# volcengine/veScale

Hardware: AMD Instinct MI355X
Metric: tokens/sec (whole node) Llama-3-8B veScale-FSDP (higher is better)
Workload: dtype bf16; 1 GPU; model=llama3_8b, global_batch=4, seq_len=8192, parallelism=fsdp1, activation_checkpointing=False, hipgraph=True

## Files before the change

### vescale_amd/ops/csrc/attention_bwd2.hip

```cpp
#include "fa32_common.h"

#define FB_D FF_D
#define FB_OWN 32
#define FB_WAVES 8
#define FB_TILE (FB_OWN * FB_WAVES)
#define FB_OTH 64
#define FB_THREADS (FB_WAVES * 64)

extern "C" __global__ void __launch_bounds__(256)
fa_bwd_preprocess(const unsigned short* __restrict__ dout,
                  const unsigned short* __restrict__ o,
                  float* __restrict__ delta, int64_t rows, int Hq, int S, int bshd) {
  const int sub = threadIdx.x & 15;
  int64_t row = (int64_t)blockIdx.x * 16 + (threadIdx.x >> 4);
  const int64_t stride = (int64_t)gridDim.x * 16;
  for (; row < rows; row += stride) {
    const unsigned short* pd = dout + row * FB_D + sub * 8;
    const unsigned short* po = o + row * FB_D + sub * 8;
    ff_shortx8 a = *reinterpret_cast<const ff_shortx8*>(pd);
    ff_shortx8 b = *reinterpret_cast<const ff_shortx8*>(po);
    float s = 0.f;
#pragma unroll
    for (int j = 0; j < 8; ++j)
      s += bf16_to_f32((unsigned short)a[j]) * bf16_to_f32((unsigned short)b[j]);
// ... 3 lines not shown
    int64_t drow = row;
    if (bshd) {
      const unsigned r = (unsigned)row, bs = r / (unsigned)Hq, h = r - bs * (unsigned)Hq;
      const unsigned bi = bs / (unsigned)S, sq = bs - bi * (unsigned)S;
      drow = ((int64_t)bi * Hq + h) * S + sq;
    }
    if (sub == 0) delta[drow] = s;
  }
}

extern "C" __global__ void __launch_bounds__(256)
fa_bwd_reduce_gqa(const unsigned short* __restrict__ part,
                  unsigned short* __restrict__ out,
                  int B, int Hq, int Hkv, int64_t SD) {
  int group = Hq / Hkv;
  int64_t total = (int64_t)B * Hkv * SD;
  int64_t i0 = (int64_t)(blockIdx.x * 256 + threadIdx.x) * 8;
  int64_t stride = (int64_t)gridDim.x * 256 * 8;
  for (int64_t i = i0; i < total; i += stride) {
    int64_t bh = i / SD;
    int64_t off = i % SD;
    int64_t b = bh / Hkv;
    int64_t hk = bh % Hkv;
    float acc[8] = {0, 0, 0, 0, 0, 0, 0, 0};
#pragma unroll 4
    for (int g = 0; g < group; ++g) {
      const unsigned short* p =
          part + ((b * Hq + hk * group + g) * SD) + off;
      ff_shortx8 v = *reinterpret_cast<const ff_shortx8*>(p);
#pragma unroll
      for (int j = 0; j < 8; ++j) acc[j] += bf16_to_f32((unsigned short)v[j]);
    }
    ff_shortx8 o;
#pragma unroll
    for (int j = 0; j < 8; ++j) o[j] = (short)f32_to_bf16(acc[j]);
    *reinterpret_cast<ff_shortx8*>(out + i) = o;
  }
}

extern "C" __global__ void __launch_bounds__(FB_THREADS, 2)
fa2_dq_bf16(const unsigned short* __restrict__ q,
            const unsigned short* __restrict__ k,
            const unsigned short* __restrict__ v,
            const unsigned short* __restrict__ dout,
            const float* __restrict__ lse,
            const float* __restrict__ delta,
            unsigned short* __restrict__ dq,
            int B, int Hq, int Hkv, int S, float scale, int bshd) {
  __shared__ unsigned short lk[FB_OTH * FB_D];
  __shared__ unsigned short lv[FB_OTH * FB_D];
  __shared__ unsigned short ldo[FB_TILE * FB_D];

  const ff_ctx c = ff_prologue(Hq, Hkv, S);
  const int tid = c.tid, wave = c.wave, l31 = c.l31, half = c.half;
  const int qt = (int)gridDim.x - 1 - c.tile;
  const int64_t qbase = c.qbase, kbase = c.kbase;
  const int q0 = qt * FB_TILE + wave * FB_OWN;
  const int my_q = q0 + l31;
  const float scale2 = scale * FF_LOG2E;

  const int64_t lrow = c.rbase + my_q;
  const float lse2 = lse[lrow] * FF_LOG2E;
  const float dlt = delta[lrow];

  ff_shortx8 qf[8];
  ff_row_frags(q + qbase + (int64_t)my_q * FB_D, qf, half);
  const ff_rows dorow = ff_o_rows(c, Hq, S, bshd);
  ff_stage_rows<FB_TILE, FB_THREADS>(
      dout + dorow.base + (int64_t)qt * FB_TILE * dorow.stride, dorow.stride, ldo, tid);

  ff_floatx16 dqacc[4];
#pragma unroll
  for (int i = 0; i < 4; ++i) dqacc[i] = (ff_floatx16)(0.f);

  const int last_kv = min((qt + 1) * (FB_TILE / FB_OTH), S / FB_OTH);
  const unsigned short* kg = k + kbase;
  const unsigned short* vg = v + kbase;

  for (int jkv = 0; jkv < last_kv; ++jkv) {
    const int kv0 = jkv * FB_OTH;
    const bool active = (kv0 <= q0 + FB_OWN - 1);
    const bool need_mask = (kv0 + FB_OTH - 1 > q0);
    __syncthreads();
    ff_stage<FB_OTH, FB_THREADS>(kg + (int64_t)kv0 * FB_D, lk, tid);
    ff_stage<FB_OTH, FB_THREADS>(vg + (int64_t)kv0 * FB_D, lv, tid);
    __syncthreads();

    if (active) {
      ff_floatx16 st[2], dp[2];
#pragma unroll
      for (int s2 = 0; s2 < 2; ++s2) {
        st[s2] = (ff_floatx16)(0.f);
        dp[s2] = (ff_floatx16)(0.f);
      }
#pragma unroll
      for (int s2 = 0; s2 < 2; ++s2)
#pragma unroll
        for (int ks = 0; ks < 8; ++ks) {
          ff_shortx8 kfr = ff_afrag(lk, s2, ks, l31, half);
          st[s2] = __builtin_amdgcn_mfma_f32_32x32x16_bf16(kfr, qf[ks], st[s2], 0, 0, 0);
          ff_shortx8 vfr = ff_afrag(lv, s2, ks, l31, half);
          ff_shortx8 dof = ff_bfrag(ldo, wave * FB_OWN + l31, ks, half);
          dp[s2] = __builtin_amdgcn_mfma_f32_32x32x16_bf16(vfr, dof, dp[s2], 0, 0, 0);
        }
#pragma unroll
      for (int s2 = 0; s2 < 2; ++s2)
#pragma unroll
        for (int r = 0; r < 16; ++r) {
          int kv = ff_drow(kv0 + s2 * 32, r, half);
          float x = st[s2][r] * scale2 - lse2;
          if (need_mask && kv > my_q) x = -INFINITY;
          float p = __builtin_amdgcn_exp2f(x);
          st[s2][r] = p * (dp[s2][r] - dlt);
        }
      ff_shortx8 pb[4];
      ff_relayout(st, pb, half);
#pragma unroll
      for (int ds = 0; ds < 4; ++ds) {
        ff_shortx4 t[4][2];
        ff_tr_read8(lk, ds, tid, l31, half, t);
#pragma unroll
        for (int ks = 0; ks < 4; ++ks)
          dqacc[ds] = __builtin_amdgcn_mfma_f32_32x32x16_bf16(
              ff_cat(t[ks][0], t[ks][1]), pb[ks], dqacc[ds], 0, 0, 0);
      }
    }
  }

  ff_store_row(dq + qbase + (int64_t)my_q * FB_D, dqacc, scale, half);
}

template <bool DK>
DEV void fa2_dv_dk_t(const unsigned short* __restrict__ q,
                     const unsigned short* __restrict__ k,
                     const unsigned short* __restrict__ v,
                     const unsigned short* __restrict__ dout,
                     const float* __restrict__ lse,
                     const float* __restrict__ delta,
                     unsigned short* __restrict__ out_part,
                     int Hq, int Hkv, int S, float scale, int bshd) {
  __shared__ unsigned short lq[FB_OTH * FB_D];
  __shared__ unsigned short ldo[FB_OTH * FB_D];
  __shared__ float llse[FB_OTH];
  __shared__ float ldelta[FB_OTH];

  const ff_ctx c = ff_prologue(Hq, Hkv, S);
  const int tid = c.tid, wave = c.wave, l31 = c.l31, half = c.half;
  const int64_t qbase = c.qbase, kbase = c.kbase;
  const int kvB = c.tile * FB_TILE;
  const int kv0w = kvB + wave * FB_OWN;
  const int my_kv = kv0w + l31;
  const float scale2 = scale * FF_LOG2E;

  ff_shortx8 kf[8], vf[DK ? 8 : 1];
  {
    const unsigned short* kg = k + kbase + (int64_t)my_kv * FB_D;
    const unsigned short* vg = DK ? v + kbase + (int64_t)my_kv * FB_D : nullptr;
#pragma unroll
    for (int ks = 0; ks < 8; ++ks) {
      kf[ks] = ff_row_frag(kg, ks, half);
      if constexpr (DK) vf[ks] = ff_row_frag(vg, ks, half);
    }
  }

  ff_floatx16 acc[4];
#pragma unroll
  for (int i = 0; i < 4; ++i) acc[i] = (ff_floatx16)(0.f);

  const int jq0 = kvB / FB_OTH;
  const int n_jq = S / FB_OTH;
  const float* lseg = lse + c.rbase;
  const float* dltg = DK ? delta + c.rbase : nullptr;
  const ff_rows dorow = ff_o_rows(c, Hq, S, bshd);

  for (int jq = jq0; jq < n_jq; ++jq) {
    const int qt0 = jq * FB_OTH;
    const bool active = (qt0 + FB_OTH - 1 >= kv0w);
    const bool need_mask = (qt0 < kv0w + FB_OWN - 1);
    __syncthreads();
    ff_stage<FB_OTH, FB_THREADS>(q + qbase + (int64_t)qt0 * FB_D, lq, tid);
    ff_stage_rows<FB_OTH, FB_THREADS>(dout + dorow.base + (int64_t)qt0 * dorow.stride,
                                      dorow.stride, ldo, tid);
    if (tid < FB_OTH) {
      llse[tid] = lseg[qt0 + tid] * FF_LOG2E;
      if constexpr (DK) ldelta[tid] = dltg[qt0 + tid];
    }
    __syncthreads();

    if (active) {
      ff_floatx16 st[2], dp[DK ? 2 : 1];
#pragma unroll
      for (int s2 = 0; s2 < 2; ++s2) {
        st[s2] = (ff_floatx16)(0.f);
        if constexpr (DK) dp[s2] = (ff_floatx16)(0.f);
      }
#pragma unroll
      for (int s2 = 0; s2 < 2; ++s2)
#pragma unroll
        for (int ks = 0; ks < 8; ++ks) {
          ff_shortx8 qfr = ff_afrag(lq, s2, ks, l31, half);
          st[s2] = __builtin_amdgcn_mfma_f32_32x32x16_bf16(qfr, kf[ks], st[s2], 0, 0, 0);
          if constexpr (DK) {
            ff_shortx8 dofr = ff_afrag(ldo, s2, ks, l31, half);
            dp[s2] = __builtin_amdgcn_mfma_f32_32x32x16_bf16(dofr, vf[ks], dp[s2], 0, 0, 0);
          }
        }
#pragma unroll
      for (int s2 = 0; s2 < 2; ++s2)
#pragma unroll
        for (int r = 0; r < 16; ++r) {
          int qrow = ff_drow(s2 * 32, r, half);
          float x = st[s2][r] * scale2 - llse[qrow];
          if (need_mask && qt0 + qrow < my_kv) x = -INFINITY;
          float p = __builtin_amdgcn_exp2f(x);
          if constexpr (DK) st[s2][r] = p * (dp[s2][r] - ldelta[qrow]);
          else st[s2][r] = p;
        }
      ff_shortx8 pb[4];
      ff_relayout(st, pb, half);
#pragma unroll
      for (int ds = 0; ds < 4; ++ds) {
        ff_shortx4 t[4][2];
        ff_tr_read8(DK ? lq : ldo, ds, tid, l31, half, t);
#pragma unroll
        for (int ks = 0; ks < 4; ++ks)
          acc[ds] = __builtin_amdgcn_mfma_f32_32x32x16_bf16(
              ff_cat(t[ks][0], t[ks][1]), pb[ks], acc[ds], 0, 0, 0);
      }
    }
  }

  unsigned short* og = out_part + qbase + (int64_t)my_kv * FB_D;
  ff_store_row<DK>(og, acc, scale, half);
}

extern "C" __global__ void __launch_bounds__(FB_THREADS, 2)
fa2_dv_bf16(const unsigned short* __restrict__ q,
            const unsigned short* __restrict__ k,
            const unsigned short* __restrict__ dout,
            const float* __restrict__ lse,
            unsigned short* __restrict__ dv_part,
            int B, int Hq, int Hkv, int S, float scale, int bshd) {
  fa2_dv_dk_t<false>(q, k, nullptr, dout, lse, nullptr, dv_part, Hq, Hkv, S, scale, bshd);
}

extern "C" __global__ void __launch_bounds__(FB_THREADS, 2)
fa2_dk_bf16(const unsigned short* __restrict__ q,
            const unsigned short* __restrict__ k,
            const unsigned short* __restrict__ v,
            const unsigned short* __restrict__ dout,
            const float* __restrict__ lse,
            const float* __restrict__ delta,
            unsigned short* __restrict__ dk_part,
            int B, int Hq, int Hkv, int S, float scale, int bshd) {
  fa2_dv_dk_t<true>(q, k, v, dout, lse, delta, dk_part, Hq, Hkv, S, scale, bshd);
}

#define FD_WAVES 4
#define FD_THREADS (FD_WAVES * 64)
#define FD_TILE (FD_WAVES * FB_OWN)

extern "C" __global__ void __launch_bounds__(FD_THREADS, 1)
fa2_dvdk_bf16(const unsigned short* __restrict__ q,
              const unsigned short* __restrict__ k,
              const unsigned short* __restrict__ v,
              const unsigned short* __restrict__ dout,
              const float* __restrict__ lse,
              const float* __restrict__ delta,
              unsigned short* __restrict__ dv_part,
              unsigned short* __restrict__ dk_part,
              int B, int Hq, int Hkv, int S, float scale) {
  __shared__ unsigned short lq[FB_OTH * FB_D];
// ... 23 lines not shown

  {
    const unsigned short* kg = k + kbase + (int64_t)kvB * FB_D;
    const unsigned short* vg = v + kbase + (int64_t)kvB * FB_D;
#pragma unroll
    for (int j = 0; j < FF_STAGE_CHUNKS(FD_TILE, FD_THREADS); ++j) {
      const int e = ff_chunk<FD_THREADS>(j, tid);
      ff_chunk_store(ff_chunk_load(kg, e), lk, e);
      ff_chunk_store(ff_chunk_load(vg, e), lv, e);
    }
  }

  ff_floatx16 dvacc[4], dkacc[4];
#pragma unroll
  for (int i = 0; i < 4; ++i) {
    dvacc[i] = (ff_floatx16)(0.f);
    dkacc[i] = (ff_floatx16)(0.f);
  }

  const int jq0 = kvB / FB_OTH;
  const int n_jq = S / FB_OTH;
  const float* lseg = lse + ((int64_t)b * Hq + h) * S;
  const float* dltg = delta + ((int64_t)b * Hq + h) * S;

  for (int jq = jq0; jq < n_jq; ++jq) {
    const int qt0 = jq * FB_OTH;
    const bool active = (qt0 + FB_OTH - 1 >= kv0w);
    const bool need_mask = (qt0 < kv0w + FB_OWN - 1);
    __syncthreads();
    ff_stage<FB_OTH, FD_THREADS>(q + qbase + (int64_t)qt0 * FB_D, lq, tid);
    ff_stage<FB_OTH, FD_THREADS>(dout + qbase + (int64_t)qt0 * FB_D, ldo, tid);
    const float lse_reg = lseg[qt0 + lane] * FF_LOG2E;
    const float dlt_reg = dltg[qt0 + lane];
    __syncthreads();

    if (active) {
      ff_floatx16 st[2], dp[2];
#pragma unroll
      for (int s2 = 0; s2 < 2; ++s2) {
        st[s2] = (ff_floatx16)(0.f);
        dp[s2] = (ff_floatx16)(0.f);
      }
#pragma unroll
      for (int s2 = 0; s2 < 2; ++s2)
#pragma unroll
        for (int ks = 0; ks < 8; ++ks) {
          ff_shortx8 kfr = ff_bfrag(lk, myrow, ks, half);
          ff_shortx8 qfr = ff_afrag(lq, s2, ks, l31, half);
          st[s2] = __builtin_amdgcn_mfma_f32_32x32x16_bf16(qfr, kfr, st[s2], 0, 0, 0);
          ff_shortx8 vfr = ff_bfrag(lv, myrow, ks, half);
          ff_shortx8 dofr = ff_afrag(ldo, s2, ks, l31, half);
          dp[s2] = __builtin_amdgcn_mfma_f32_32x32x16_bf16(dofr, vfr, dp[s2], 0, 0, 0);
        }
#pragma unroll
      for (int s2 = 0; s2 < 2; ++s2)
#pragma unroll
        for (int r = 0; r < 16; ++r) {
          int qrow = ff_drow(s2 * 32, r, half);
          float l2 = __int_as_float(
              __builtin_amdgcn_ds_bpermute(qrow * 4, __float_as_int(lse_reg)));
          float x = st[s2][r] * scale2 - l2;
          if (need_mask && qt0 + qrow < my_kv) x = -INFINITY;
          st[s2][r] = __builtin_amdgcn_exp2f(x);
        }
      {
        ff_shortx8 pb[4];
        ff_relayout(st, pb, half);
#pragma unroll
        for (int ds = 0; ds < 4; ++ds) {
          ff_shortx4 t[4][2];
          ff_tr_read8(ldo, ds, tid, l31, half, t);
#pragma unroll
          for (int ks = 0; ks < 4; ++ks)
            dvacc[ds] = __builtin_amdgcn_mfma_f32_32x32x16_bf16(
                ff_cat(t[ks][0], t[ks][1]), pb[ks], dvacc[ds], 0, 0, 0);
        }
      }
#pragma unroll
      for (int s2 = 0; s2 < 2; ++s2)
#pragma unroll
        for (int r = 0; r < 16; ++r) {
          int qrow = ff_drow(s2 * 32, r, half);
          float dl = __int_as_float(
              __builtin_amdgcn_ds_bpermute(qrow * 4, __float_as_int(dlt_reg)));
          st[s2][r] = st[s2][r] * (dp[s2][r] - dl);
        }
      {
        ff_shortx8 pb[4];
        ff_relayout(st, pb, half);
#pragma unroll
        for (int ds = 0; ds < 4; ++ds) {
          ff_shortx4 t[4][2];
          ff_tr_read8(lq, ds, tid, l31, half, t);
#pragma unroll
          for (int ks = 0; ks < 4; ++ks)
            dkacc[ds] = __builtin_amdgcn_mfma_f32_32x32x16_bf16(
                ff_cat(t[ks][0], t[ks][1]), pb[ks], dkacc[ds], 0, 0, 0);
        }
      }
    }
  }

  unsigned short* ogv = dv_part + qbase + (int64_t)my_kv * FB_D;
  unsigned short* ogk = dk_part + qbase + (int64_t)my_kv * FB_D;
#pragma unroll
  for (int ds = 0; ds < 4; ++ds)
#pragma unroll
    for (int r = 0; r < 16; ++r) {
      ff_store_elem(ogv, ds, r, half, dvacc[ds][r]);
      ff_store_elem(ogk, ds, r, half, dkacc[ds][r] * scale);
    }
}
```

### vescale_amd/ops/csrc/attention_fwd.hip

```cpp
#include "fa32_common.h"

#define FF_QBLK 32
#define FF_WAVES 4
#define FF_QTILE (FF_QBLK * FF_WAVES)
#define FF_KV 64
#define FF_THREADS (FF_WAVES * 64)
#define FF_CHUNKS FF_STAGE_CHUNKS(FF_KV, FF_THREADS)

template <int MODE>
DEV void fa_fwd_t(const unsigned short* __restrict__ q,
            const unsigned short* __restrict__ k,
            const unsigned short* __restrict__ v,
            unsigned short* __restrict__ out,
            float* __restrict__ lse,
            int B, int Hq, int Hkv, int S, float scale, int out_bshd) {
  __shared__ unsigned short lk[2][FF_KV * FF_D];
  __shared__ unsigned short lv[2][FF_KV * FF_D];

  const ff_ctx c = ff_prologue(Hq, Hkv, S);
  const int tid = c.tid, lane = c.lane, l31 = c.l31, half = c.half;
  const int qt = c.tile;
  const int q0 = qt * FF_QTILE + c.wave * FF_QBLK;
  const int my_q = q0 + l31;
  const float scale2 = (MODE == 5) ? scale : scale * FF_LOG2E;

  ff_shortx8 qf[8];
  ff_row_frags(q + c.qbase + (int64_t)my_q * FF_D, qf, half);

  float m_run = -INFINITY;
  float l_run = 0.f;
  ff_floatx16 oacc[4];
#pragma unroll
  for (int i = 0; i < 4; ++i) oacc[i] = (ff_floatx16)(0.f);

  const int n_kv = (qt + 1) * (FF_QTILE / FF_KV);
  const int last_kv = min(n_kv, S / FF_KV);

  const unsigned short* kg = k + c.kbase;
  const unsigned short* vg = v + c.kbase;
  ff_shortx8 kreg[FF_CHUNKS], vreg[FF_CHUNKS];
#pragma unroll
  for (int j = 0; j < FF_CHUNKS; ++j) {
    const int e = ff_chunk<FF_THREADS>(j, tid);
    kreg[j] = ff_chunk_load(kg, e);
    vreg[j] = ff_chunk_load(vg, e);
  }
#pragma unroll
  for (int j = 0; j < FF_CHUNKS; ++j) {
    const int e = ff_chunk<FF_THREADS>(j, tid);
    ff_chunk_store(kreg[j], lk[0], e);
    ff_chunk_store(vreg[j], lv[0], e);
  }
  __syncthreads();

  for (int jkv = 0; jkv < last_kv; ++jkv) {
    const int kv0 = jkv * FF_KV;
    const int buf = jkv & 1;
    const bool have_next = (jkv + 1 < last_kv);
    const bool active = (MODE == 4) || (kv0 <= q0 + FF_QBLK - 1);
    const bool need_mask = (MODE == 4) || (kv0 + FF_KV - 1 > q0);
    if (have_next) {
      const unsigned short* kn = kg + (int64_t)(kv0 + FF_KV) * FF_D;
      const unsigned short* vn = vg + (int64_t)(kv0 + FF_KV) * FF_D;
#pragma unroll
      for (int j = 0; j < FF_CHUNKS; ++j) {
        const int e = ff_chunk<FF_THREADS>(j, tid);
        kreg[j] = ff_chunk_load(kn, e);
        vreg[j] = ff_chunk_load(vn, e);
      }
    }

    if (active) {
    ff_floatx16 st[2];
#pragma unroll
    for (int s2 = 0; s2 < 2; ++s2) st[s2] = (ff_floatx16)(MODE == 3 ? 1e-3f : 0.f);
    if constexpr (MODE != 3)
#pragma unroll
    for (int s2 = 0; s2 < 2; ++s2) {
#pragma unroll
      for (int ks = 0; ks < 8; ++ks) {
        ff_shortx8 kf = ff_afrag(lk[buf], s2, ks, l31, half);
        st[s2] = __builtin_amdgcn_mfma_f32_32x32x16_bf16(kf, qf[ks], st[s2], 0, 0, 0);
      }
    }

    if constexpr (MODE == 1 || MODE == 3) {
      l_run += 1.f; m_run = 0.f;
    } else {
    float pmax = -INFINITY;
    if (need_mask) {
#pragma unroll
      for (int s2 = 0; s2 < 2; ++s2)
#pragma unroll
        for (int r = 0; r < 16; ++r) {
          int kv = ff_drow(kv0 + s2 * 32, r, half);
          float x = (kv <= my_q) ? st[s2][r] * scale2 : -INFINITY;
          st[s2][r] = x;
          pmax = fmaxf(pmax, x);
        }
    } else {
#pragma unroll
      for (int s2 = 0; s2 < 2; ++s2)
#pragma unroll
        for (int r = 0; r < 16; ++r) {
          float x = st[s2][r] * scale2;
          st[s2][r] = x;
          pmax = fmaxf(pmax, x);
        }
    }
    pmax = fmaxf(pmax, __int_as_float(ff_swap_other(__float_as_int(pmax), half)));
    float m_new = fmaxf(m_run, pmax);
    bool dead = false;
    if constexpr (MODE == 4) dead = (m_new == -INFINITY);
    float corr;
    if constexpr (MODE == 5) corr = __expf(m_run - m_new);
    else corr = __builtin_amdgcn_exp2f(m_run - m_new);
    if (dead) { corr = 1.f; m_new = m_run; }
    float psum = 0.f;
#pragma unroll
    for (int s2 = 0; s2 < 2; ++s2)
#pragma unroll
      for (int r = 0; r < 16; ++r) {
        float p;
        if (dead) p = 0.f;
        else if constexpr (MODE == 5) p = (st[s2][r] == -INFINITY) ? 0.f : __expf(st[s2][r] - m_new);
        else p = __builtin_amdgcn_exp2f(st[s2][r] - m_new);
        st[s2][r] = p;
        psum += p;
      }
    psum += __int_as_float(ff_swap_other(__float_as_int(psum), half));
    l_run = l_run * corr + psum;
    m_run = m_new;

#pragma unroll
    for (int ds = 0; ds < 4; ++ds)
#pragma unroll
      for (int r = 0; r < 16; ++r) oacc[ds][r] *= corr;
    }

    if constexpr (MODE == 2) {
#pragma unroll
      for (int r = 0; r < 16; ++r) oacc[0][r] += st[0][r] + st[1][r];
    } else {
    ff_shortx8 pb[4];
    ff_relayout(st, pb, half);
#pragma unroll
    for (int ds = 0; ds < 4; ++ds) {
      ff_shortx4 t[4][2];
      ff_tr_read8(lv[buf], ds, lane, l31, half, t);
#pragma unroll
      for (int ks = 0; ks < 4; ++ks)
        oacc[ds] = __builtin_amdgcn_mfma_f32_32x32x16_bf16(
            ff_cat(t[ks][0], t[ks][1]), pb[ks], oacc[ds], 0, 0, 0);
    }
    }
    }

    if (have_next) {
#pragma unroll
      for (int j = 0; j < FF_CHUNKS; ++j) {
        const int e = ff_chunk<FF_THREADS>(j, tid);
        ff_chunk_store(kreg[j], lk[buf ^ 1], e);
        ff_chunk_store(vreg[j], lv[buf ^ 1], e);
      }
    }
    __syncthreads();
  }

  float inv_l = (l_run > 0.f) ? 1.0f / l_run : 0.f;
  const ff_rows orow = ff_o_rows(c, Hq, S, out_bshd);
  ff_store_row(out + orow.base + (int64_t)my_q * orow.stride, oacc, inv_l, half);
  if (half == 0)
    lse[c.rbase + my_q] = m_run * (MODE == 5 ? 1.0f : FF_LN2) + __logf(l_run);
}

extern "C" __global__ void __launch_bounds__(FF_THREADS, 2)
fa_fwd_bf16(const unsigned short* q, const unsigned short* k,
            const unsigned short* v, unsigned short* out, float* lse,
            int B, int Hq, int Hkv, int S, float scale, int out_bshd) {
  fa_fwd_t<0>(q, k, v, out, lse, B, Hq, Hkv, S, scale, out_bshd);
}
extern "C" __global__ void __launch_bounds__(FF_THREADS, 2)
fa_fwd_bf16_ab1(const unsigned short* q, const unsigned short* k,
                const unsigned short* v, unsigned short* out, float* lse,
                int B, int Hq, int Hkv, int S, float scale, int out_bshd) {
  fa_fwd_t<1>(q, k, v, out, lse, B, Hq, Hkv, S, scale, out_bshd);
}
extern "C" __global__ void __launch_bounds__(FF_THREADS, 2)
fa_fwd_bf16_ab2(const unsigned short* q, const unsigned short* k,
                const unsigned short* v, unsigned short* out, float* lse,
                int B, int Hq, int Hkv, int S, float scale, int out_bshd) {
  fa_fwd_t<2>(q, k, v, out, lse, B, Hq, Hkv, S, scale, out_bshd);
}
extern "C" __global__ void __launch_bounds__(FF_THREADS, 2)
fa_fwd_bf16_ab3(const unsigned short* q, const unsigned short* k,
                const unsigned short* v, unsigned short* out, float* lse,
                int B, int Hq, int Hkv, int S, float scale, int out_bshd) {
  fa_fwd_t<3>(q, k, v, out, lse, B, Hq, Hkv, S, scale, out_bshd);
// ... 14 lines not shown
```

### vescale_amd/ops/csrc/extension.hip

```cpp
#include <torch/extension.h>
#include <ATen/cuda/CUDAContext.h>
#include <c10/cuda/CUDAException.h>
#include <c10/cuda/CUDAGuard.h>

#include "rmsnorm.hip"
#include "rope.hip"
#include "rope_qkv.hip"
#include "swiglu.hip"
#include "adamw.hip"
#include "cross_entropy.hip"
#include "philox_random.hip"
#include "gemm.hip"
#include "gemm8.hip"
#include "attention_fwd.hip"
#include "attention_bwd2.hip"
#include "attention_gen.hip"

#include <climits>
#include <sstream>
#include <vector>

namespace {

constexpr auto BF16 = at::kBFloat16;
// ... 471 lines not shown
std::vector<at::Tensor> fa_fwd_impl(const Binding& b, int64_t mode, at::Tensor q,
                                    at::Tensor k, at::Tensor v, double scale,
                                    bool out_bshd) {
  FaShape s = fa_check(b, FF_QTILE, q, k, v);
  TORCH_CHECK(!out_bshd || (int64_t)s.Hq * FF_D <= INT_MAX, b.fn,
              ": Hq * 128 must fit int in the [B,S,Hq,D] layout");
  auto out = out_bshd ? at::empty({s.B, s.S, s.Hq, FF_D}, q.options()) : at::empty_like(q);
  auto lse = at::empty({s.B, s.Hq, s.S}, q.options().dtype(F32));
  decltype(&fa_fwd_bf16) kerns[] = {fa_fwd_bf16,     fa_fwd_bf16_ab1, fa_fwd_bf16_ab2,
                                    fa_fwd_bf16_ab3, fa_fwd_bf16_ab4, fa_fwd_bf16_ab5};
  b.launch(kerns[mode], dim3(s.S / FF_QTILE, s.Hq, s.B), FF_THREADS, bf16(q), bf16(k), bf16(v),
           bf16_mut(out), lse.data_ptr<float>(), s.B, s.Hq, s.Hkv, s.S, (float)scale,
           out_bshd ? 1 : 0);
  return {out, lse};
}

std::vector<at::Tensor> fa_fwd(at::Tensor q, at::Tensor k, at::Tensor v, double scale,
                               bool out_bshd) {
  return fa_fwd_impl(Binding("fa_fwd", "q", q), 0, q, k, v, scale, out_bshd);
}

std::vector<at::Tensor> fa_fwd_ablate(at::Tensor q, at::Tensor k, at::Tensor v,
                                      double scale, int64_t mode) {
  TORCH_CHECK(mode >= 0 && mode <= 5, "fa_fwd_ablate: mode = ", mode,
              " must be in 0..5");
  return fa_fwd_impl(Binding("fa_fwd_ablate", "q", q), mode, q, k, v, scale, false);
}

at::Tensor fa_bwd_delta(const Binding& b, const FaShape& s, const at::Tensor& dout,
                        const at::Tensor& o, bool bshd = false) {
  auto delta = at::empty({s.B, s.Hq, s.S}, o.options().dtype(F32));
  int64_t rows = (int64_t)s.B * s.Hq * s.S;
  b.launch(fa_bwd_preprocess, grid_for(rows, 1, 4096), 256, bf16(dout), bf16(o),
           delta.data_ptr<float>(), rows, s.Hq, s.S, bshd ? 1 : 0);
  return delta;
}

at::Tensor fa_bwd_reduce(const Binding& b, const FaShape& s, const at::Tensor& part) {
  if (s.Hkv == s.Hq) return part;
  auto out = at::empty({s.B, s.Hkv, s.S, FF_D}, part.options());
  int64_t SD = (int64_t)s.S * FF_D;
  b.launch(fa_bwd_reduce_gqa, grid_for((int64_t)s.B * s.Hkv * SD / 8, 256), 256,
           bf16(part), bf16_mut(out), s.B, s.Hq, s.Hkv, SD);
  return out;
}

std::vector<at::Tensor> fa_bwd2(at::Tensor q, at::Tensor k, at::Tensor v, at::Tensor o,
                                at::Tensor dout, at::Tensor lse, double scale,
                                bool fused_dvdk, bool bshd) {
  Binding b("fa_bwd2", "q", q);
  TORCH_CHECK(!(bshd && fused_dvdk), "fa_bwd2: the fused dv+dk kernel reads [B,Hq,S,D] ",
              "only: bshd=True needs fused_dvdk=False");
  FaShape s = fa_check(b, FB_TILE, q, k, v, o, dout, lse, bshd);
  auto delta = fa_bwd_delta(b, s, dout, o, bshd);
  auto dq = at::empty_like(q);
  dim3 grid(s.S / FB_TILE, s.Hq, s.B);
  b.launch(fa2_dq_bf16, grid, FB_THREADS, bf16(q), bf16(k), bf16(v), bf16(dout),
           lse.data_ptr<float>(), delta.data_ptr<float>(), bf16_mut(dq), s.B, s.Hq,
           s.Hkv, s.S, (float)scale, bshd ? 1 : 0);
  auto dv_part = at::empty_like(q);
  auto dk_part = at::empty_like(q);
  if (fused_dvdk) {
    b.launch(fa2_dvdk_bf16, dim3(s.S / FD_TILE, s.Hq, s.B), FD_THREADS, bf16(q),
             bf16(k), bf16(v), bf16(dout), lse.data_ptr<float>(),
             delta.data_ptr<float>(), bf16_mut(dv_part), bf16_mut(dk_part), s.B, s.Hq,
             s.Hkv, s.S, (float)scale);
  } else {
    b.launch(fa2_dv_bf16, grid, FB_THREADS, bf16(q), bf16(k), bf16(dout),
             lse.data_ptr<float>(), bf16_mut(dv_part), s.B, s.Hq, s.Hkv, s.S,
             (float)scale, bshd ? 1 : 0);
    b.launch(fa2_dk_bf16, grid, FB_THREADS, bf16(q), bf16(k), bf16(v), bf16(dout),
             lse.data_ptr<float>(), delta.data_ptr<float>(), bf16_mut(dk_part), s.B,
             s.Hq, s.Hkv, s.S, (float)scale, bshd ? 1 : 0);
  }
  return {dq, fa_bwd_reduce(b, s, dk_part), fa_bwd_reduce(b, s, dv_part)};
}

struct FaGenShape { int B, Hq, Hkv, Sq, Sk, D, shift; bool seg; };

FaGenShape fa_gen_check(const Binding& b, const at::Tensor& q, const at::Tensor& k,
                        const at::Tensor& v, bool causal, int64_t shift,
                        const OptTensor& q_seg, const OptTensor& kv_seg) {
  TORCH_CHECK(q.dim() == 4 && k.dim() == 4 && v.dim() == 4,
              b.fn, ": q, k, v must be [B, H, S, D]");
  int64_t D = q.size(3);
  TORCH_CHECK(D == 64 || D == 128, b.fn, ": fa_gen supports head_dim 64 and 128");
  TORCH_CHECK(k.size(1) >= 1 && q.size(1) % k.size(1) == 0,
              b.fn, ": Hq must be a multiple of Hkv");
  TORCH_CHECK(q.size(2) >= 1 && k.size(2) >= 1, b.fn, ": Sq and Sk must be >= 1");
  TORCH_CHECK(q.size(0) >= 1 && q.size(0) <= 65535 && q.size(1) <= 65535,
              b.fn, ": B and Hq must be in [1, 65535]");
  TORCH_CHECK(q.size(2) + k.size(2) < (int64_t)1 << 30, b.fn, ": sequence too long");
  TORCH_CHECK(causal || shift == 0, b.fn, ": shift needs causal");
  TORCH_CHECK(q_seg.has_value() == kv_seg.has_value(), b.fn,
              ": q_seg and kv_seg must be given together");
  b.arg("q", q, BF16);
  b.arg("k", k, BF16, {q.size(0), -1, -1, D});
  b.arg("v", v, BF16, k.sizes());
  b.arg("q_seg", q_seg, I32, {q.size(0), q.size(2)});
  b.arg("kv_seg", kv_seg, I32, {q.size(0), k.size(2)});
  int64_t sh = std::max<int64_t>(-q.size(2), std::min<int64_t>(k.size(2), shift));
  return {(int)q.size(0), (int)q.size(1), (int)k.size(1), (int)q.size(2),
          (int)k.size(2), (int)D, (int)sh, q_seg.has_value()};
}

#define FA_GEN_KERNEL(kernel, D) ((D) == 64 ? kernel<64> : kernel<128>)
// ... 136 lines not shown
           need_mask ? mask.data_ptr<unsigned char>() : nullptr, d, n, (uint64_t)seed,
           (uint64_t)philox_offset, (float)p);
  if (need_mask) return {out, mask};
  return {out};
}

}

PYBIND11_MODULE(TORCH_EXTENSION_NAME, m) {
  m.def("rmsnorm_fwd", &rmsnorm_fwd);
  m.def("rmsnorm_bwd", &rmsnorm_bwd, pybind11::arg("dy"), pybind11::arg("x"),
        pybind11::arg("w"), pybind11::arg("rrms"),
        pybind11::arg("dres") = pybind11::none());
  m.def("rmsnorm_res_fwd", &rmsnorm_res_fwd);
  m.def("rope", &rope);
  m.def("rope_qkv_fwd", &rope_qkv_fwd);
  m.def("rope_qkv_bwd", &rope_qkv_bwd);
  m.def("swiglu_fwd", &swiglu_fwd);
  m.def("swiglu_bwd", &swiglu_bwd);
  m.def("swiglu_packed_fwd", &swiglu_packed_fwd);
  m.def("swiglu_packed_bwd", &swiglu_packed_bwd);
  m.def("ce_fwd", &ce_fwd, pybind11::arg("logits"), pybind11::arg("target"),
        pybind11::arg("ignore_index"), pybind11::arg("vocab_start") = 0,
        pybind11::arg("vocab_total") = -1);
  m.def("ce_bwd", &ce_bwd, pybind11::arg("logits"), pybind11::arg("target"),
        pybind11::arg("lse"), pybind11::arg("dloss"), pybind11::arg("ignore_index"),
        pybind11::arg("inplace"), pybind11::arg("vocab_start") = 0,
        pybind11::arg("vocab_total") = -1);
  m.def("adamw_step", &adamw_step);
  m.def("l2norm_sq", &l2norm_sq);
  m.def("scale_", &scale_);
  m.def("gemm_tn", &gemm_tn, pybind11::arg("a"), pybind11::arg("b"), pybind11::arg("variant") = 0);
  m.def("gemm_tn8", &gemm_tn8, pybind11::arg("a"), pybind11::arg("b"), pybind11::arg("mode") = 0);
  m.def("fa_bwd", &fa_bwd);
  m.def("fa_bwd2", &fa_bwd2, pybind11::arg("q"), pybind11::arg("k"), pybind11::arg("v"),
        pybind11::arg("o"), pybind11::arg("dout"), pybind11::arg("lse"),
        pybind11::arg("scale"), pybind11::arg("fused_dvdk"), pybind11::arg("bshd") = false);
  m.def("fa_fwd", &fa_fwd, pybind11::arg("q"), pybind11::arg("k"), pybind11::arg("v"),
        pybind11::arg("scale"), pybind11::arg("out_bshd") = false);
  m.def("fa_fwd_ablate", &fa_fwd_ablate);
  m.def("fa_gen_fwd", &fa_gen_fwd, pybind11::arg("q"), pybind11::arg("k"),
        pybind11::arg("v"), pybind11::arg("scale"), pybind11::arg("causal"),
        pybind11::arg("shift"), pybind11::arg("q_seg") = pybind11::none(),
        pybind11::arg("kv_seg") = pybind11::none());
  m.def("fa_gen_bwd", &fa_gen_bwd, pybind11::arg("q"), pybind11::arg("k"),
        pybind11::arg("v"), pybind11::arg("o"), pybind11::arg("dout"),
        pybind11::arg("lse"), pybind11::arg("dlse"), pybind11::arg("scale"),
        pybind11::arg("causal"), pybind11::arg("shift"),
        pybind11::arg("q_seg") = pybind11::none(),
        pybind11::arg("kv_seg") = pybind11::none());
  m.def("permlane_probe", &permlane_probe);
  m.def("mfma32_probe", &mfma32_probe);
  m.def("tr_probe", &tr_probe);
  m.def("philox_uniform_", &philox_fill<false>);
  m.def("philox_normal_", &philox_fill<true>);
  m.def("philox_dropout", &philox_dropout);
}
```

### vescale_amd/ops/csrc/fa32_common.h

```cpp
#pragma once
#include "common.h"
#include "fa32_lds_map.h"

#define FF_D 128
#define FF_LOG2E 1.44269504088896340736f
#define FF_LN2 0.69314718055994530942f

typedef float ff_floatx16 __attribute__((ext_vector_type(16)));
typedef short ff_shortx4 __attribute__((ext_vector_type(4)));
typedef short ff_shortx8 __attribute__((ext_vector_type(8)));
typedef int ff_intx4 __attribute__((ext_vector_type(4)));
typedef __attribute__((address_space(3))) const unsigned short* ff_lds_p;

DEV int ff_swap_other(int x, int half) {
  auto r = __builtin_amdgcn_permlane32_swap(x, x, false, false);
  return half ? r[0] : r[1];
}

DEV void ff_xcd_remap(int& bx, int& by, int& bz) {
  int gx = gridDim.x, gy = gridDim.y;
  int nwg = gx * gy * (int)gridDim.z;
  if ((nwg & 7) != 0) return;
  int f = bx + gx * (by + gy * bz);
  f = (f & 7) * (nwg >> 3) + (f >> 3);
// ... 39 lines not shown
  return *reinterpret_cast<const ff_shortx8*>(g + e);
}
DEV void ff_chunk_store(ff_shortx8 v, unsigned short* l, int e) {
  *reinterpret_cast<ff_shortx8*>((char*)l + ff_map_chunk_byte(e)) = v;
}
template <int ROWS, int THREADS>
DEV void ff_stage(const unsigned short* __restrict__ g, unsigned short* l, int tid) {
#pragma unroll
  for (int j = 0; j < FF_STAGE_CHUNKS(ROWS, THREADS); ++j) {
    const int e = ff_chunk<THREADS>(j, tid);
    ff_chunk_store(ff_chunk_load(g, e), l, e);
  }
}

struct ff_rows {
  int64_t base;
  int stride;
};
DEV ff_rows ff_o_rows(const ff_ctx& c, int Hq, int S, int bshd) {
  ff_rows r;
  r.stride = bshd ? Hq * FF_D : FF_D;
  r.base = bshd ? ((int64_t)c.b * S * Hq + c.h) * FF_D : c.qbase;
  return r;
}

template <int ROWS, int THREADS>
DEV void ff_stage_rows(const unsigned short* __restrict__ g, int stride, unsigned short* l,
                       int tid) {
#pragma unroll
  for (int j = 0; j < FF_STAGE_CHUNKS(ROWS, THREADS); ++j) {
    const int e = ff_chunk<THREADS>(j, tid);
    const int ge = (e / FF_D) * stride + (e % FF_D);
    ff_chunk_store(ff_chunk_load(g, ge), l, e);
  }
}

DEV ff_shortx8 ff_afrag(const unsigned short* l, int s2, int ks, int l31, int half) {
  return *reinterpret_cast<const ff_shortx8*>((const char*)l +
                                              ff_map_frag(s2 * 32 + l31, ks, half));
}

DEV ff_shortx8 ff_bfrag(const unsigned short* l, int row, int ks, int half) {
  return *reinterpret_cast<const ff_shortx8*>((const char*)l + ff_map_frag(row, ks, half));
}

DEV ff_shortx8 ff_row_frag(const unsigned short* __restrict__ row, int ks, int half) {
  return *reinterpret_cast<const ff_shortx8*>(row + ks * 16 + half * 8);
}
DEV void ff_row_frags(const unsigned short* __restrict__ row, ff_shortx8 (&f)[8], int half) {
#pragma unroll
  for (int ks = 0; ks < 8; ++ks) f[ks] = ff_row_frag(row, ks, half);
}

DEV void ff_relayout(const ff_floatx16 st[2], ff_shortx8 pb[4], int half) {
#pragma unroll
  for (int s2 = 0; s2 < 2; ++s2) {
#pragma unroll
    for (int g = 0; g < 2; ++g) {
      unsigned lo0, lo1, hi0, hi1;
      asm volatile("v_cvt_pk_bf16_f32 %0, %1, %2" : "=v"(lo0)
                   : "v"(st[s2][g * 8 + 0]), "v"(st[s2][g * 8 + 1]));
      asm volatile("v_cvt_pk_bf16_f32 %0, %1, %2" : "=v"(lo1)
                   : "v"(st[s2][g * 8 + 2]), "v"(st[s2][g * 8 + 3]));
      asm volatile("v_cvt_pk_bf16_f32 %0, %1, %2" : "=v"(hi0)
                   : "v"(st[s2][g * 8 + 4]), "v"(st[s2][g * 8 + 5]));
      asm volatile("v_cvt_pk_bf16_f32 %0, %1, %2" : "=v"(hi1)
                   : "v"(st[s2][g * 8 + 6]), "v"(st[s2][g * 8 + 7]));
      int p0 = ff_swap_other((int)lo0, half);
      int p1 = ff_swap_other((int)lo1, half);
      int p2 = ff_swap_other((int)hi0, half);
      int p3 = ff_swap_other((int)hi1, half);
      ff_intx4 frag;
      if (half == 0) {
        frag = (ff_intx4){(int)lo0, (int)lo1, p0, p1};
      } else {
        frag = (ff_intx4){p2, p3, (int)hi0, (int)hi1};
      }
      pb[s2 * 2 + g] = *reinterpret_cast<ff_shortx8*>(&frag);
    }
  }
}

DEV void ff_tr_read8(const unsigned short* tile, int ds, int l15, int l31, int half,
                     ff_shortx4 (&t)[4][2]) {
  static_assert(FF_MAP_KS_BYTES == 4096, "the offset: immediates below step 16 rows");
  const int a0 = ff_map_tr(ds, l15, l31, half, 0);
  const int a1 = ff_map_tr(ds, l15, l31, half, 1);
  ff_lds_p b0 = (ff_lds_p)((const char*)tile + a0);
  ff_lds_p b1 = (ff_lds_p)((const char*)tile + a1);
  asm volatile(
      "ds_read_b64_tr_b16 %0, %8 offset:0\n\t"
      "ds_read_b64_tr_b16 %1, %9 offset:0\n\t"
      "ds_read_b64_tr_b16 %2, %8 offset:4096\n\t"
      "ds_read_b64_tr_b16 %3, %9 offset:4096\n\t"
      "ds_read_b64_tr_b16 %4, %8 offset:8192\n\t"
      "ds_read_b64_tr_b16 %5, %9 offset:8192\n\t"
      "ds_read_b64_tr_b16 %6, %8 offset:12288\n\t"
      "ds_read_b64_tr_b16 %7, %9 offset:12288\n\t"
      "s_waitcnt lgkmcnt(0)"
      : "=&v"(t[0][0]), "=&v"(t[0][1]), "=&v"(t[1][0]), "=&v"(t[1][1]),
        "=&v"(t[2][0]), "=&v"(t[2][1]), "=&v"(t[3][0]), "=&v"(t[3][1])
      : "v"(b0), "v"(b1));
}

DEV ff_shortx8 ff_cat(const ff_shortx4 a, const ff_shortx4 b) {
  ff_shortx8 r;
#pragma unroll
  for (int x = 0; x < 4; ++x) { r[x] = a[x]; r[4 + x] = b[x]; }
  return r;
}

DEV void ff_store_elem(unsigned short* __restrict__ row, int ds, int r, int half, float x) {
  row[ff_drow(ds * 32, r, half)] = f32_to_bf16(x);
}
template <bool SCALE = true>
DEV void ff_store_row(unsigned short* __restrict__ row, const ff_floatx16 (&acc)[4],
                      float mul, int half) {
#pragma unroll
  for (int ds = 0; ds < 4; ++ds)
#pragma unroll
    for (int r = 0; r < 16; ++r) {
      if constexpr (SCALE) ff_store_elem(row, ds, r, half, acc[ds][r] * mul);
      else ff_store_elem(row, ds, r, half, acc[ds][r]);
    }
}
```

### vescale_amd/ops/csrc/probes.hip

```cpp
#include "fa32_common.h"

extern "C" __global__ void permlane_probe_kernel(int* out) {
  int x = (int)threadIdx.x;
  auto r = __builtin_amdgcn_permlane32_swap(x, x, false, false);
  out[threadIdx.x] = (r[0] << 16) | (r[1] & 0xFFFF);
}

extern "C" __global__ void mfma32_probe_kernel(float* out) {
  typedef short sx8 __attribute__((ext_vector_type(8)));
  typedef float fx16 __attribute__((ext_vector_type(16)));
  int lane = threadIdx.x & 63;
  int l31 = lane & 31, half = lane >> 5;
  sx8 af, bf, a1, bj, ak, bk;
  for (int e = 0; e < 8; ++e) {
    int k = half * 8 + e;
    af[e] = (short)f32_to_bf16((float)((k == 0) ? l31 : 0));
    bf[e] = (short)f32_to_bf16((float)((k == 0) ? 1 : 0));
    a1[e] = bf[e];
    bj[e] = (short)f32_to_bf16((float)((k == 0) ? l31 : 0));
    ak[e] = (short)f32_to_bf16((float)((k == 5) ? 1 : 0));
    bk[e] = (short)f32_to_bf16((float)((k == 5) ? l31 : 0));
  }
  fx16 z = (fx16)(0.f);
  fx16 d1 = __builtin_amdgcn_mfma_f32_32x32x16_bf16(af, bf, z, 0, 0, 0);
  fx16 d2 = __builtin_amdgcn_mfma_f32_32x32x16_bf16(a1, bj, z, 0, 0, 0);
  fx16 d3 = __builtin_amdgcn_mfma_f32_32x32x16_bf16(ak, bk, z, 0, 0, 0);
  for (int r = 0; r < 16; ++r) {
    out[0 * 64 * 16 + lane * 16 + r] = d1[r];
    out[1 * 64 * 16 + lane * 16 + r] = d2[r];
    out[2 * 64 * 16 + lane * 16 + r] = d3[r];
  }
}

extern "C" __global__ void tr_probe_kernel(unsigned short* out) {
  __shared__ unsigned short lvp[64 * FF_D];
  const int lane = threadIdx.x;
#pragma unroll
  for (int j = 0; j < FF_STAGE_CHUNKS(64, 64); ++j) {
    const int e = ff_chunk<64>(j, lane);
    ff_shortx8 vv;
#pragma unroll
    for (int x = 0; x < 8; ++x) vv[x] = (short)(e + x);
    ff_chunk_store(vv, lvp, e);
  }
  __syncthreads();
#pragma unroll
  for (int ds = 0; ds < 4; ++ds) {
    ff_shortx4 t[4][2];
    ff_tr_read8(lvp, ds, lane, lane & 31, lane >> 5, t);
#pragma unroll
    for (int ks = 0; ks < 4; ++ks)
      *reinterpret_cast<ff_shortx8*>(out + ((ds * 4 + ks) * 64 + lane) * 8) =
          ff_cat(t[ks][0], t[ks][1]);
  }
}

namespace {

at::Tensor probe_out(at::IntArrayRef sizes, at::ScalarType dtype) {
  return at::empty(sizes, at::TensorOptions().dtype(dtype).device(at::kCUDA));
}

at::Tensor permlane_probe() {
  auto out = probe_out({64}, at::kInt);
  Binding("permlane_probe", "out", out).launch(permlane_probe_kernel, 1, 64, out.data_ptr<int>());
  return out;
}

at::Tensor mfma32_probe() {
  auto out = probe_out({3, 64, 16}, at::kFloat);
  Binding("mfma32_probe", "out", out).launch(mfma32_probe_kernel, 1, 64, out.data_ptr<float>());
  return out;
}

at::Tensor tr_probe() {
  auto out = probe_out({4, 4, 64, 8}, at::kShort);
  Binding("tr_probe", "out", out).launch(tr_probe_kernel, 1, 64, bf16_mut(out));
  return out;
}

}
```

Baseline: 19020 tokens/s.

## Streamline flash-attention relayout, masking, and MFMA scheduling in fwd/bwd kernels

Replaces the half-dependent lane swap in the P relayout with permlane32_swap pairs, so each lane no longer needs two swaps plus a branch. The causal mask moves out of the exp loop into a separate pass that applies it only on diagonal tiles. The dV kernel preloads all Q fragments and interleaves LDS reads with MFMAs using sched_group_barrier. Smaller changes: the wave id is made scalar with readfirstlane, the dq store index is recomputed with mbcnt, an explicit waitcnt is added before the forward barrier, and a scale check and a relayout probe are added. These cut VALU and cross-lane work in attention backward and forward, at the cost of inline asm and scheduling hints that tie the code to specific hardware behavior.

```diff
diff --git a/vescale_amd/ops/csrc/attention_bwd2.hip b/vescale_amd/ops/csrc/attention_bwd2.hip
--- a/vescale_amd/ops/csrc/attention_bwd2.hip
+++ b/vescale_amd/ops/csrc/attention_bwd2.hip
@@ -79,7 +79,8 @@
   __shared__ unsigned short ldo[FB_TILE * FB_D];
 
   const ff_ctx c = ff_prologue(Hq, Hkv, S);
-  const int tid = c.tid, wave = c.wave, l31 = c.l31, half = c.half;
+  const int tid = c.tid, l31 = c.l31, half = c.half;
+  const int wave = __builtin_amdgcn_readfirstlane(c.wave);
   const int qt = (int)gridDim.x - 1 - c.tile;
   const int64_t qbase = c.qbase, kbase = c.kbase;
   const int q0 = qt * FB_TILE + wave * FB_OWN;
@@ -130,18 +131,16 @@
           ff_shortx8 dof = ff_bfrag(ldo, wave * FB_OWN + l31, ks, half);
           dp[s2] = __builtin_amdgcn_mfma_f32_32x32x16_bf16(vfr, dof, dp[s2], 0, 0, 0);
         }
+      if (need_mask) ff_mask<true>(st, my_q - kv0 - 4 * half);
 #pragma unroll
       for (int s2 = 0; s2 < 2; ++s2)
 #pragma unroll
         for (int r = 0; r < 16; ++r) {
-          int kv = ff_drow(kv0 + s2 * 32, r, half);
-          float x = st[s2][r] * scale2 - lse2;
-          if (need_mask && kv > my_q) x = -INFINITY;
-          float p = __builtin_amdgcn_exp2f(x);
+          float p = __builtin_amdgcn_exp2f(st[s2][r] * scale2 - lse2);
           st[s2][r] = p * (dp[s2][r] - dlt);
         }
       ff_shortx8 pb[4];
-      ff_relayout(st, pb, half);
+      ff_relayout(st, pb);
 #pragma unroll
       for (int ds = 0; ds < 4; ++ds) {
         ff_shortx4 t[4][2];
@@ -154,7 +153,10 @@
     }
   }
 
-  ff_store_row(dq + qbase + (int64_t)my_q * FB_D, dqacc, scale, half);
+  int elane;
+  asm volatile("v_mbcnt_lo_u32_b32 %0, -1, 0\n\tv_mbcnt_hi_u32_b32 %0, -1, %0" : "=v"(elane));
+  const int e_q = qt * FB_TILE + wave * FB_OWN + (elane & 31);
+  ff_store_row(dq + qbase + (int64_t)e_q * FB_D, dqacc, scale, elane >> 5);
 }
 
 template <bool DK>
@@ -221,30 +223,43 @@
         st[s2] = (ff_floatx16)(0.f);
         if constexpr (DK) dp[s2] = (ff_floatx16)(0.f);
       }
-#pragma unroll
-      for (int s2 = 0; s2 < 2; ++s2)
-#pragma unroll
-        for (int ks = 0; ks < 8; ++ks) {
-          ff_shortx8 qfr = ff_afrag(lq, s2, ks, l31, half);
-          st[s2] = __builtin_amdgcn_mfma_f32_32x32x16_bf16(qfr, kf[ks], st[s2], 0, 0, 0);
-          if constexpr (DK) {
+      if constexpr (!DK) {
+        ff_shortx8 qfr[16];
+#pragma unroll
+        for (int i = 0; i < 16; ++i) qfr[i] = ff_afrag(lq, i & 1, i >> 1, l31, half);
+#pragma unroll
+        for (int i = 0; i < 16; ++i)
+          st[i & 1] = __builtin_amdgcn_mfma_f32_32x32x16_bf16(qfr[i], kf[i >> 1], st[i & 1], 0, 0, 0);
+        __builtin_amdgcn_sched_group_barrier(0x100, 4, 0);
+#pragma unroll
+        for (int i = 0; i < 12; ++i) {
+          __builtin_amdgcn_sched_group_barrier(0x008, 1, 0);
+          __builtin_amdgcn_sched_group_barrier(0x100, 1, 0);
+        }
+        __builtin_amdgcn_sched_group_barrier(0x008, 4, 0);
+      } else {
+#pragma unroll
+        for (int s2 = 0; s2 < 2; ++s2)
+#pragma unroll
+          for (int ks = 0; ks < 8; ++ks) {
+            ff_shortx8 qfr = ff_afrag(lq, s2, ks, l31, half);
+            st[s2] = __builtin_amdgcn_mfma_f32_32x32x16_bf16(qfr, kf[ks], st[s2], 0, 0, 0);
             ff_shortx8 dofr = ff_afrag(ldo, s2, ks, l31, half);
             dp[s2] = __builtin_amdgcn_mfma_f32_32x32x16_bf16(dofr, vf[ks], dp[s2], 0, 0, 0);
           }
-        }
+      }
+      if (need_mask) ff_mask<false>(st, my_kv - qt0 - 4 * half);
 #pragma unroll
       for (int s2 = 0; s2 < 2; ++s2)
 #pragma unroll
         for (int r = 0; r < 16; ++r) {
           int qrow = ff_drow(s2 * 32, r, half);
-          float x = st[s2][r] * scale2 - llse[qrow];
-          if (need_mask && qt0 + qrow < my_kv) x = -INFINITY;
-          float p = __builtin_amdgcn_exp2f(x);
+          float p = __builtin_amdgcn_exp2f(st[s2][r] * scale2 - llse[qrow]);
           if constexpr (DK) st[s2][r] = p * (dp[s2][r] - ldelta[qrow]);
           else st[s2][r] = p;
         }
       ff_shortx8 pb[4];
-      ff_relayout(st, pb, half);
+      ff_relayout(st, pb);
 #pragma unroll
       for (int ds = 0; ds < 4; ++ds) {
         ff_shortx4 t[4][2];
@@ -374,6 +389,7 @@
           ff_shortx8 dofr = ff_afrag(ldo, s2, ks, l31, half);
           dp[s2] = __builtin_amdgcn_mfma_f32_32x32x16_bf16(dofr, vfr, dp[s2], 0, 0, 0);
         }
+      if (need_mask) ff_mask<false>(st, my_kv - qt0 - 4 * half);
 #pragma unroll
       for (int s2 = 0; s2 < 2; ++s2)
 #pragma unroll
@@ -381,13 +397,11 @@
           int qrow = ff_drow(s2 * 32, r, half);
           float l2 = __int_as_float(
               __builtin_amdgcn_ds_bpermute(qrow * 4, __float_as_int(lse_reg)));
-          float x = st[s2][r] * scale2 - l2;
-          if (need_mask && qt0 + qrow < my_kv) x = -INFINITY;
-          st[s2][r] = __builtin_amdgcn_exp2f(x);
+          st[s2][r] = __builtin_amdgcn_exp2f(st[s2][r] * scale2 - l2);
         }
       {
         ff_shortx8 pb[4];
-        ff_relayout(st, pb, half);
+        ff_relayout(st, pb);
 #pragma unroll
         for (int ds = 0; ds < 4; ++ds) {
           ff_shortx4 t[4][2];
@@ -409,7 +423,7 @@
         }
       {
         ff_shortx8 pb[4];
-        ff_relayout(st, pb, half);
+        ff_relayout(st, pb);
 #pragma unroll
         for (int ds = 0; ds < 4; ++ds) {
           ff_shortx4 t[4][2];
diff --git a/vescale_amd/ops/csrc/attention_fwd.hip b/vescale_amd/ops/csrc/attention_fwd.hip
--- a/vescale_amd/ops/csrc/attention_fwd.hip
+++ b/vescale_amd/ops/csrc/attention_fwd.hip
@@ -51,6 +51,7 @@
     ff_chunk_store(kreg[j], lk[0], e);
     ff_chunk_store(vreg[j], lv[0], e);
   }
+  __builtin_amdgcn_s_waitcnt(0x0F70);
   __syncthreads();
 
   for (int jkv = 0; jkv < last_kv; ++jkv) {
@@ -143,7 +144,7 @@
       for (int r = 0; r < 16; ++r) oacc[0][r] += st[0][r] + st[1][r];
     } else {
     ff_shortx8 pb[4];
-    ff_relayout(st, pb, half);
+    ff_relayout(st, pb);
 #pragma unroll
     for (int ds = 0; ds < 4; ++ds) {
       ff_shortx4 t[4][2];
diff --git a/vescale_amd/ops/csrc/extension.hip b/vescale_amd/ops/csrc/extension.hip
--- a/vescale_amd/ops/csrc/extension.hip
+++ b/vescale_amd/ops/csrc/extension.hip
@@ -547,6 +547,8 @@
   TORCH_CHECK(!(bshd && fused_dvdk), "fa_bwd2: the fused dv+dk kernel reads [B,Hq,S,D] ",
               "only: bshd=True needs fused_dvdk=False");
   FaShape s = fa_check(b, FB_TILE, q, k, v, o, dout, lse, bshd);
+  TORCH_CHECK(scale > 0 && std::isfinite(scale), b.fn, ": scale = ", scale,
+              " must be positive and finite");
   auto delta = fa_bwd_delta(b, s, dout, o, bshd);
   auto dq = at::empty_like(q);
   dim3 grid(s.S / FB_TILE, s.Hq, s.B);
@@ -789,6 +791,7 @@
   m.def("permlane_probe", &permlane_probe);
   m.def("mfma32_probe", &mfma32_probe);
   m.def("tr_probe", &tr_probe);
+  m.def("_relayout_probe", &relayout_probe, pybind11::arg("x"));
   m.def("philox_uniform_", &philox_fill<false>);
   m.def("philox_normal_", &philox_fill<true>);
   m.def("philox_dropout", &philox_dropout);
diff --git a/vescale_amd/ops/csrc/fa32_common.h b/vescale_amd/ops/csrc/fa32_common.h
--- a/vescale_amd/ops/csrc/fa32_common.h
+++ b/vescale_amd/ops/csrc/fa32_common.h
@@ -115,33 +115,37 @@
   for (int ks = 0; ks < 8; ++ks) f[ks] = ff_row_frag(row, ks, half);
 }
 
-DEV void ff_relayout(const ff_floatx16 st[2], ff_shortx8 pb[4], int half) {
+DEV unsigned ff_cvt_pk(float a, float b) {
+  unsigned w;
+  asm volatile("v_cvt_pk_bf16_f32 %0, %1, %2" : "=v"(w) : "v"(a), "v"(b));
+  return w;
+}
+DEV void ff_relayout(const ff_floatx16 st[2], ff_shortx8 pb[4]) {
 #pragma unroll
   for (int s2 = 0; s2 < 2; ++s2) {
 #pragma unroll
     for (int g = 0; g < 2; ++g) {
-      unsigned lo0, lo1, hi0, hi1;
-      asm volatile("v_cvt_pk_bf16_f32 %0, %1, %2" : "=v"(lo0)
-                   : "v"(st[s2][g * 8 + 0]), "v"(st[s2][g * 8 + 1]));
-      asm volatile("v_cvt_pk_bf16_f32 %0, %1, %2" : "=v"(lo1)
-                   : "v"(st[s2][g * 8 + 2]), "v"(st[s2][g * 8 + 3]));
-      asm volatile("v_cvt_pk_bf16_f32 %0, %1, %2" : "=v"(hi0)
-                   : "v"(st[s2][g * 8 + 4]), "v"(st[s2][g * 8 + 5]));
-      asm volatile("v_cvt_pk_bf16_f32 %0, %1, %2" : "=v"(hi1)
-                   : "v"(st[s2][g * 8 + 6]), "v"(st[s2][g * 8 + 7]));
-      int p0 = ff_swap_other((int)lo0, half);
-      int p1 = ff_swap_other((int)lo1, half);
-      int p2 = ff_swap_other((int)hi0, half);
-      int p3 = ff_swap_other((int)hi1, half);
-      ff_intx4 frag;
-      if (half == 0) {
-        frag = (ff_intx4){(int)lo0, (int)lo1, p0, p1};
-      } else {
-        frag = (ff_intx4){p2, p3, (int)hi0, (int)hi1};
-      }
+      const unsigned lo0 = ff_cvt_pk(st[s2][g * 8 + 0], st[s2][g * 8 + 1]);
+      const unsigned lo1 = ff_cvt_pk(st[s2][g * 8 + 2], st[s2][g * 8 + 3]);
+      const unsigned hi0 = ff_cvt_pk(st[s2][g * 8 + 4], st[s2][g * 8 + 5]);
+      const unsigned hi1 = ff_cvt_pk(st[s2][g * 8 + 6], st[s2][g * 8 + 7]);
+      auto w0 = __builtin_amdgcn_permlane32_swap(lo0, hi0, false, false);
+      auto w1 = __builtin_amdgcn_permlane32_swap(lo1, hi1, false, false);
+      ff_intx4 frag = (ff_intx4){(int)w0[0], (int)w1[0], (int)w0[1], (int)w1[1]};
       pb[s2 * 2 + g] = *reinterpret_cast<ff_shortx8*>(&frag);
     }
   }
+}
+
+template <bool ABOVE>
+DEV void ff_mask(ff_floatx16 (&st)[2], int lim) {
+#pragma unroll
+  for (int s2 = 0; s2 < 2; ++s2)
+#pragma unroll
+    for (int r = 0; r < 16; ++r) {
+      const int row = ff_drow(s2 * 32, r, 0);
+      if (ABOVE ? row > lim : row < lim) st[s2][r] = -INFINITY;
+    }
 }
 
 DEV void ff_tr_read8(const unsigned short* tile, int ds, int l15, int l31, int half,
diff --git a/vescale_amd/ops/csrc/probes.hip b/vescale_amd/ops/csrc/probes.hip
--- a/vescale_amd/ops/csrc/probes.hip
+++ b/vescale_amd/ops/csrc/probes.hip
@@ -55,6 +55,48 @@
   }
 }
 
+DEV void ff_relayout_ref(const ff_floatx16 st[2], ff_shortx8 pb[4], int half) {
+#pragma unroll
+  for (int s2 = 0; s2 < 2; ++s2) {
+#pragma unroll
+    for (int g = 0; g < 2; ++g) {
+      const unsigned lo0 = ff_cvt_pk(st[s2][g * 8 + 0], st[s2][g * 8 + 1]);
+      const unsigned lo1 = ff_cvt_pk(st[s2][g * 8 + 2], st[s2][g * 8 + 3]);
+      const unsigned hi0 = ff_cvt_pk(st[s2][g * 8 + 4], st[s2][g * 8 + 5]);
+      const unsigned hi1 = ff_cvt_pk(st[s2][g * 8 + 6], st[s2][g * 8 + 7]);
+      int p0 = ff_swap_other((int)lo0, half);
+      int p1 = ff_swap_other((int)lo1, half);
+      int p2 = ff_swap_other((int)hi0, half);
+      int p3 = ff_swap_other((int)hi1, half);
+      ff_intx4 frag;
+      if (half == 0) {
+        frag = (ff_intx4){(int)lo0, (int)lo1, p0, p1};
+      } else {
+        frag = (ff_intx4){p2, p3, (int)hi0, (int)hi1};
+      }
+      pb[s2 * 2 + g] = *reinterpret_cast<ff_shortx8*>(&frag);
+    }
+  }
+}
+
+extern "C" __global__ void relayout_probe_kernel(const float* __restrict__ in,
+                                                 unsigned short* __restrict__ out) {
+  const int lane = threadIdx.x;
+  ff_floatx16 st[2];
+#pragma unroll
+  for (int s2 = 0; s2 < 2; ++s2)
+#pragma unroll
+    for (int r = 0; r < 16; ++r) st[s2][r] = in[lane * 32 + s2 * 16 + r];
+  ff_shortx8 ref[4], got[4];
+  ff_relayout_ref(st, ref, lane >> 5);
+  ff_relayout(st, got);
+#pragma unroll
+  for (int f = 0; f < 4; ++f) {
+    *reinterpret_cast<ff_shortx8*>(out + ((0 * 64 + lane) * 4 + f) * 8) = ref[f];
+    *reinterpret_cast<ff_shortx8*>(out + ((1 * 64 + lane) * 4 + f) * 8) = got[f];
+  }
+}
+
 namespace {
 
 at::Tensor probe_out(at::IntArrayRef sizes, at::ScalarType dtype) {
@@ -79,4 +121,12 @@
   return out;
 }
 
+at::Tensor relayout_probe(at::Tensor x) {
+  Binding b("_relayout_probe", "x", x);
+  b.arg("x", x, F32, {64, 32});
+  auto out = at::empty({2, 64, 4, 8}, x.options().dtype(at::kShort));
+  b.launch(relayout_probe_kernel, 1, 64, x.data_ptr<float>(), bf16_mut(out));
+  return out;
 }
+
+}
```

New measurement: 19740 tokens/s, median of 6. 1.04x the previous value.
